# nh2/lz4-frame-conduit

Hardware: AMD Instinct MI355X
Metric: GiB/s end-to-end (compress+decompress), 4 MiB blocks, 1/2/4/8 GPUs vs liblz4 (higher is better)
Workload: dtype u8

## Files before the change

### lz4_frame_conduit_amd/csrc/encode.cuh

```cuda
#pragma once
#include <type_traits>
#include "common.cuh"

namespace lz4f {

constexpr uint32_t MFLIMIT = 12, LASTLIT = 5, MINMATCH = 4;
constexpr uint32_t ENC_POOL_SHORT = 0x200u;

struct ChunkInfo {
    uint32_t nrec;
    uint32_t first_lit;
    uint32_t tail_lit;
    uint32_t body_size;
    uint32_t carry_in;
    uint32_t flags;
    uint64_t out_off;
};

struct EncGeom {
    uint64_t src_size;
    uint64_t first_off;
    uint32_t write_endmark;
    uint32_t block_size;
    uint32_t chunk_size;
    uint32_t chunks_per_block;
    uint32_t n_blocks;
    uint32_t n_chunks;
    uint32_t linked;
    uint32_t block_checksum;
    uint32_t header_size;
    uint8_t  header[20];
    uint32_t max_rec_per_chunk;
    uint64_t rec_pool;
    uint32_t seed_stride;
    uint32_t tiles_per_wg;
    uint32_t e1_solo;
    uint32_t hc_attempts;
    uint32_t hc_lazy;
};

struct EncPlace {
    uint64_t bstart, bend_abs;
    uint64_t cs_abs, ce_abs;
    uint64_t low_abs;
    uint64_t rd_end;
};
__device__ __forceinline__ bool enc_place(const EncGeom& g, uint32_t chunk, EncPlace& pl)
{
    const uint32_t blk = chunk / g.chunks_per_block, cib = chunk % g.chunks_per_block;
    pl.bstart = g.first_off + (uint64_t)blk * g.block_size;
    pl.bend_abs = (pl.bstart + g.block_size < g.src_size) ? pl.bstart + g.block_size : g.src_size;
    pl.cs_abs = pl.bstart + (uint64_t)cib * g.chunk_size;
    if (pl.cs_abs >= pl.bend_abs) return false;
    pl.ce_abs = (pl.cs_abs + g.chunk_size < pl.bend_abs) ? pl.cs_abs + g.chunk_size : pl.bend_abs;
    pl.low_abs = g.linked ? 0 : pl.bstart;
    pl.rd_end = g.src_size;
    return true;
}

__device__ __forceinline__ unsigned long long* rec_ctl(const uint64_t* recs) { return (unsigned long long*)recs; }
__device__ __forceinline__ uint32_t* rec_offs(const uint64_t* recs) { return (uint32_t*)(recs + 8); }
__host__ __device__ __forceinline__ uint64_t rec_pool_at(uint32_t n_chunks) { return 8 + (((uint64_t)n_chunks + 1 + 15) / 16) * 8; }
__device__ __forceinline__ uint64_t* rec_pool_of(const uint64_t* recs, const EncGeom& g) { return (uint64_t*)recs + rec_pool_at(g.n_chunks); }

__device__ __forceinline__ uint32_t len_ext_bytes(uint32_t v) { return v >= 15 ? (v - 15) / 255 + 1 : 0; }
__device__ __forceinline__ uint32_t seq_size(uint32_t lit, uint32_t mlen)
{
    return 1 + len_ext_bytes(lit) + lit + 2 + len_ext_bytes(mlen - MINMATCH);
}
__device__ __forceinline__ uint64_t pack_rec(uint32_t lit, uint32_t mlen, uint32_t off)
{
    return (uint64_t)lit | ((uint64_t)mlen << 24) | ((uint64_t)off << 48);
}

struct uint4_ua { uint32_t x, y, z, w; } __attribute__((packed, aligned(1)));
__device__ __forceinline__ uint32_t ld32(const uint8_t* p) { return *(const u32_ua*)p; }
typedef uint64_t u64_ua __attribute__((aligned(1)));
__device__ __forceinline__ uint64_t ld64_guard(const uint8_t* p, const uint8_t* end)
{
    if (p + 8 <= end) return *(const u64_ua*)p;
    uint64_t v = 0;
    for (int i = 0; i < 8; i++) if (p + i < end) v |= (uint64_t)p[i] << (8 * i);
    return v;
}

constexpr uint32_t E1_TILE = 65536, E1_RING = 2 * E1_TILE, E1_RMASK = E1_RING - 1;
#ifndef E1_SLICE_BYTES
#define E1_SLICE_BYTES 128
#endif
constexpr uint32_t E1_SLICE = E1_SLICE_BYTES, E1_NSLICE = E1_TILE / E1_SLICE, E1_REC_PER_SLICE = E1_SLICE / MINMATCH;
constexpr uint32_t E1_HASH_LOG = 13;
#ifndef E1_WAVES
#define E1_WAVES 16
#endif
#ifdef E1_DEBUG
#define E1DBG(...) __VA_ARGS__
#else
#define E1DBG(...)
#endif
#define E1_DBG_AT (((uint64_t)gridDim.x) * (2 * E1_NSLICE * E1_REC_PER_SLICE))
struct alignas(16) E1Shared {
    uint16_t table[1u << E1_HASH_LOG];
    uint8_t  tags[1u << E1_HASH_LOG];
    uint32_t s_end[2][E1_NSLICE];
    uint8_t  s_n[2][E1_NSLICE];
    uint32_t next, cov;
    uint32_t first;
    uint32_t cur[16];
    uint32_t pieces[2];
    uint32_t mode, hits;
    uint32_t tail_d[2];
    uint32_t idle[64];
    alignas(16) uint8_t ring[E1_RING + 16];
};
static_assert(sizeof(E1Shared) <= 163840, "one workgroup per CU");
static_assert(64 * E1_WAVES >= E1_NSLICE, "a thread per slice when the lists are merged");
#ifndef E1_GRAB
#define E1_GRAB 8
#endif
#ifndef E1_GRAB_D
#define E1_GRAB_D 1
// ... 768 lines not shown
        const uint32_t nr = (c < nch && usable && !(e.word >> 31)) ? ci[c].nrec : 0u;
        uint32_t ts, te;
        const uint32_t ps = wave_excl_scan(nr, ts), pe = wave_excl_scan((nr + IX_STRIDE - 1) / IX_STRIDE, te);
        if (c < g.chunks_per_block) ck[c] = IxChunk{nent + pe, nseq + ps};
        const uint64_t m = __ballot(nr != 0);
        if (m) last = c0 + 63u - (uint32_t)__builtin_clzll(m);
        nseq += ts; nent += te;
    }
    if (lane == 0) {
        if (last != 0xFFFFFFFFu) { ck[last].ent_off |= 0x80000000u; nseq += 1; }
        blocks[b].nseq = nseq; blocks[b].nentries = nent;
    }
}

__global__ __launch_bounds__(1024) void k_build_index(EncGeom g, const ChunkInfo* __restrict__ info, const BlockOut* __restrict__ table,
                                                      const ResultRec* __restrict__ res, void* __restrict__ ix, uint64_t ix_capacity,
                                                      uint32_t blocks_done = 0)
{
    __shared__ uint32_t s_a[1024], s_b[1024];
    __shared__ uint32_t s_carry_a, s_carry_b;
    const uint32_t t = threadIdx.x;
    IxHeader* hd = (IxHeader*)ix;
    IxBlock* blocks = ix_blocks(ix);
    IxChunk* chunks = ix_chunks(ix, g.n_blocks);
    const size_t fixed = ix_entries_at(g.n_blocks, g.chunks_per_block);
    if (ix_capacity < fixed) { if (t == 0 && ix_capacity >= sizeof(IxHeader)) hd->magic = 0; return; }
    const bool usable = res->status == ST_OK;
    for (uint32_t b = t; b < g.n_blocks && !blocks_done; b += 1024) {
        const BlockOut e = table[b];
        const ChunkInfo* ci = info + (uint64_t)b * g.chunks_per_block;
        IxChunk* ck = chunks + (uint64_t)b * g.chunks_per_block;
        const uint32_t nch = (e.dst_size + g.chunk_size - 1) / g.chunk_size;
        uint32_t nseq = 0, nent = 0, last = 0xFFFFFFFFu;
        for (uint32_t c0 = 0; c0 < g.chunks_per_block; c0 += 8) {
            uint32_t nr[8];
#pragma unroll
            for (uint32_t k = 0; k < 8; k++) nr[k] = (c0 + k < nch) ? ci[c0 + k].nrec : 0;
#pragma unroll
            for (uint32_t k = 0; k < 8; k++) {
                const uint32_t c = c0 + k;
                if (c >= g.chunks_per_block) break;
                ck[c] = IxChunk{nent, nseq};
                if (usable && !(e.word >> 31) && nr[k]) { nseq += nr[k]; nent += (nr[k] + IX_STRIDE - 1) / IX_STRIDE; last = c; }
            }
        }
        if (last != 0xFFFFFFFFu) { ck[last].ent_off |= 0x80000000u; nseq += 1; }
        blocks[b].nseq = nseq; blocks[b].nentries = nent;
    }
    __syncthreads();
    if (t == 0) { s_carry_a = 0; s_carry_b = 0; }
    __syncthreads();
    for (uint32_t base = 0; base < g.n_blocks; base += 1024) {
        const uint32_t b = base + t;
        const uint32_t va = (b < g.n_blocks) ? blocks[b].nseq : 0, vb = (b < g.n_blocks) ? blocks[b].nentries : 0;
        s_a[t] = va; s_b[t] = vb;
        __syncthreads();
        for (uint32_t off = 1; off < 1024; off <<= 1) {
            const uint32_t aa = (t >= off) ? s_a[t - off] : 0, ab = (t >= off) ? s_b[t - off] : 0;
            __syncthreads();
            s_a[t] += aa; s_b[t] += ab;
            __syncthreads();
        }
        if (b < g.n_blocks) { blocks[b].seq_base = s_carry_a + s_a[t] - va; blocks[b].entry_base = s_carry_b + s_b[t] - vb; }
        __syncthreads();
        if (t == 1023) { s_carry_a += s_a[1023]; s_carry_b += s_b[1023]; }
        __syncthreads();
    }
    if (t == 0) {
        const bool fits = (uint64_t)s_carry_b * sizeof(IxEntry) <= ix_capacity - fixed;
        *hd = IxHeader{usable && fits ? IX_MAGIC : 0u, g.n_blocks, g.chunks_per_block, s_carry_a, s_carry_b, IX_STRIDE, g.linked ? 1u : 0u, 0u};
    }
}

__device__ __forceinline__ void emit_len_ext(uint8_t* p, uint32_t v )
{
    const uint32_t n255 = v / 255, lane = lane_id();
    for (uint32_t i = lane; i < n255; i += WAVE) p[i] = 255;
    if (lane == 0) p[n255] = (uint8_t)(v - n255 * 255);
}

#ifndef E2_V2
#define E2_V2 1
#endif
template <bool split>
__device__ __forceinline__ void emit_chunk(const uint8_t* __restrict__ src, const EncPlace& pl, const ChunkInfo& ci, const uint64_t* __restrict__ rec,
                                           uint8_t* __restrict__ dst, IxEntry* ent, const uint32_t ent_seq0, const uint32_t ent_last, const uint64_t pay0,
                                           const uint32_t blk, uint4* T0, uint4* T1, const uint32_t sub, const uint32_t nsub)
{
    const uint32_t lane = lane_id();
    const uint64_t bstart = pl.bstart, cs_abs = pl.cs_abs, ce_abs = pl.ce_abs;
    if (ci.flags & 4u) return;
    if (ci.flags & 1u) {
        uint8_t* o = dst + ci.out_off;
        const uint64_t n = ce_abs - cs_abs;
        if (sub) return;
        for (uint64_t off = 0; off < n; off += 1u << 20) {
            const uint32_t m = (uint32_t)((n - off < (1u << 20)) ? n - off : (1u << 20));
            wave_copy_disjoint(o + off, src + cs_abs + off, m);
        }
        return;
    }
    uint64_t lp_off = cs_abs - ci.carry_in;
    uint64_t o_off = ci.out_off;
    auto scan = [&](uint32_t v, uint32_t& total) -> uint32_t {
        uint32_t incl = v;
#pragma unroll
        for (int sft = 1; sft < 64; sft <<= 1) { const uint32_t t = __shfl_up(incl, sft); if ((int)lane >= sft) incl += t; }
        total = __builtin_amdgcn_readlane(incl, 63);
        return incl - v;
    };
    auto find = [&](uint32_t u) -> uint32_t {
        uint32_t j = 0;
#pragma unroll
        for (uint32_t step = 32; step; step >>= 1) { const uint32_t c = j + step; if (T0[c].x <= u) j = c; }
        return j;
    };
    auto put_ext = [&](uint8_t* q, uint32_t v ) {
        const uint32_t n255 = v / 255;
        for (uint32_t i = 0; i < n255; i++) q[i] = 255;
        q[n255] = (uint8_t)(v - n255 * 255);
    };
    if ((uint64_t)ci.nrec * 192 <= ce_abs - cs_abs) {
        uint8_t* o = dst + o_off;
        const uint8_t* lp = src + lp_off;
#if E2_V2
        for (uint32_t r0 = 0; r0 < ci.nrec; r0 += WAVE) {
            const uint32_t rl = r0 + lane;
            const uint64_t xr = rl < ci.nrec ? rec[rl] : 0ull;
            uint32_t vlit = (uint32_t)(xr & 0xFFFFFFu);
            const uint32_t vmlen = (uint32_t)((xr >> 24) & 0xFFFFFFu), voff = (uint32_t)(xr >> 48);
            if (rl == 0) vlit += ci.carry_in;
            const uint32_t vmcode = rl < ci.nrec ? vmlen - MINMATCH : 0u;
            const uint32_t vhb = 1 + len_ext_bytes(vlit), vtb = 2 + len_ext_bytes(vmcode);
            const uint32_t vtoken = ((vlit < 15 ? vlit : 15) << 4) | (vmcode < 15 ? vmcode : 15);
            const uint32_t vlrest = vlit >= 15 ? (vlit - 15) % 255 : 0u, vmrest = vmcode >= 15 ? (vmcode - 15) % 255 : 0u;
            const bool vbig = vhb > WAVE || vtb > WAVE;
            const uint32_t vp1 = (vbig ? 0u : vhb | (vtb << 8)) | (vtoken << 16) | (vlrest << 24), vp2 = voff | (vmrest << 16), vadv = vlit + vmlen;
            const uint32_t nb = ci.nrec - r0 < WAVE ? ci.nrec - r0 : WAVE;
            if constexpr (split) {
                const bool vact = rl < ci.nrec;
                uint32_t tot_sz, tot_adv;
                const uint32_t vso = scan(vact ? vhb + vlit + vtb : 0u, tot_sz), vsa = scan(vact ? vadv : 0u, tot_adv);
                for (uint32_t k = sub; k < nb; k += nsub) {
                    const uint32_t r = r0 + k;
                    const uint32_t lit = (uint32_t)__builtin_amdgcn_readlane((int)vlit, (int)k), so = (uint32_t)__builtin_amdgcn_readlane((int)vso, (int)k);
                    const uint32_t sa = (uint32_t)__builtin_amdgcn_readlane((int)vsa, (int)k);
                    const uint32_t p1 = (uint32_t)__builtin_amdgcn_readlane((int)vp1, (int)k), p2 = (uint32_t)__builtin_amdgcn_readlane((int)vp2, (int)k);
                    const uint32_t hb = p1 & 0xFFu, tb = (p1 >> 8) & 0xFFu, token = (p1 >> 16) & 0xFFu, off = p2 & 0xFFFFu;
                    uint8_t* q = o + so;
                    const uint8_t* ls = lp + sa;
                    if (ent && (r % IX_STRIDE) == 0 && lane == 0) {
                        uint32_t ns = ci.nrec - r < IX_STRIDE ? ci.nrec - r : IX_STRIDE;
                        if (ent_last && r + IX_STRIDE >= ci.nrec) ns += 1;
                        ent[r / IX_STRIDE] = IxEntry{(uint32_t)((uint64_t)(q - dst) - pay0), (uint32_t)((uint64_t)(ls - src) - bstart), ent_seq0 + r, ns | (blk << 8)};
                    }
                    if (hb) {
                        const uint32_t hi = lane < hb - 1 ? lane : hb - 1, ti = lane < tb - 1 ? lane : tb - 1;
                        q[hi] = (uint8_t)(hi == 0 ? token : hi < hb - 1 ? 255u : p1 >> 24);
                        q += hb;
                        wave_copy_disjoint(q, ls, lit);
                        q += lit;
                        q[ti] = (uint8_t)(ti == 0 ? off : ti == 1 ? off >> 8 : ti < tb - 1 ? 255u : p2 >> 16);
                    } else {
                        const uint32_t mcode = (uint32_t)__builtin_amdgcn_readlane((int)vmcode, (int)k);
                        if (lane == 0) *q = (uint8_t)token;
                        q += 1;
                        if (lit >= 15) { emit_len_ext(q, lit - 15); q += len_ext_bytes(lit); }
                        wave_copy_disjoint(q, ls, lit);
                        q += lit;
                        if (lane == 0) { q[0] = (uint8_t)off; q[1] = (uint8_t)(off >> 8); }
                        q += 2;
                        if (mcode >= 15) emit_len_ext(q, mcode - 15);
                    }
                }
                o += tot_sz; lp += tot_adv;
                continue;
            }
            for (uint32_t k = 0; k < nb; k++) {
                const uint32_t r = r0 + k;
                if (ent && (r % IX_STRIDE) == 0 && lane == 0) {
                    uint32_t ns = ci.nrec - r < IX_STRIDE ? ci.nrec - r : IX_STRIDE;
                    if (ent_last && r + IX_STRIDE >= ci.nrec) ns += 1;
                    ent[r / IX_STRIDE] = IxEntry{(uint32_t)((uint64_t)(o - dst) - pay0), (uint32_t)((uint64_t)(lp - src) - bstart), ent_seq0 + r, ns | (blk << 8)};
                }
                const uint32_t lit = (uint32_t)__builtin_amdgcn_readlane((int)vlit, (int)k), adv = (uint32_t)__builtin_amdgcn_readlane((int)vadv, (int)k);
                const uint32_t p1 = (uint32_t)__builtin_amdgcn_readlane((int)vp1, (int)k), p2 = (uint32_t)__builtin_amdgcn_readlane((int)vp2, (int)k);
                const uint32_t hb = p1 & 0xFFu, tb = (p1 >> 8) & 0xFFu, token = (p1 >> 16) & 0xFFu, off = p2 & 0xFFFFu;
                if (hb) {
                    const uint32_t hi = lane < hb - 1 ? lane : hb - 1, ti = lane < tb - 1 ? lane : tb - 1;
                    o[hi] = (uint8_t)(hi == 0 ? token : hi < hb - 1 ? 255u : p1 >> 24);
                    o += hb;
                    wave_copy_disjoint(o, lp, lit);
                    o += lit;
                    o[ti] = (uint8_t)(ti == 0 ? off : ti == 1 ? off >> 8 : ti < tb - 1 ? 255u : p2 >> 16);
                    o += tb;
                } else {
                    const uint32_t mcode = adv - lit - MINMATCH;
                    if (lane == 0) *o = (uint8_t)token;
                    o += 1;
                    if (lit >= 15) { emit_len_ext(o, lit - 15); o += len_ext_bytes(lit); }
                    wave_copy_disjoint(o, lp, lit);
                    o += lit;
                    if (lane == 0) { o[0] = (uint8_t)off; o[1] = (uint8_t)(off >> 8); }
                    o += 2;
                    if (mcode >= 15) { emit_len_ext(o, mcode - 15); o += len_ext_bytes(mcode); }
                }
                lp += adv;
            }
        }
#else
        for (uint32_t r = 0; r < ci.nrec; r++) {
            if (ent && (r % IX_STRIDE) == 0 && lane == 0) {
                uint32_t ns = ci.nrec - r < IX_STRIDE ? ci.nrec - r : IX_STRIDE;
                if (ent_last && r + IX_STRIDE >= ci.nrec) ns += 1;
                ent[r / IX_STRIDE] = IxEntry{(uint32_t)((uint64_t)(o - dst) - pay0), (uint32_t)((uint64_t)(lp - src) - bstart), ent_seq0 + r, ns | (blk << 8)};
            }
            const uint64_t x = rec[r];
            uint32_t lit = (uint32_t)(x & 0xFFFFFFu);
            const uint32_t mlen = (uint32_t)((x >> 24) & 0xFFFFFFu), off = (uint32_t)(x >> 48);
            if (r == 0) lit += ci.carry_in;
            const uint32_t mcode = mlen - MINMATCH;
// ... 73 lines not shown
                const uint8_t* a = on ? sb + (e1.x + o16) : src;
                const b16_ua t = *(const b16_ua*)a;
                pc.a = t.a; pc.b = t.b; pc.c = t.c; pc.d = t.d;
            };
            auto st = [&](const P16& pc, uint32_t dof, bool on) { if (on) *(b16_ua*)(ob + dof) = b16_ua{pc.a, pc.b, pc.c, pc.d}; };
            P16 a0, b0;
            uint32_t da0, db0;
            bool xa0, xb0;
            uint32_t base = 0;
            ld(a0, base + lane, da0, xa0); base += 64;
            for (;;) {
                const bool more_b = base < total;
                ld(b0, base + lane, db0, xb0); base += 64;
                st(a0, da0, xa0);
                if (!more_b) break;
                const bool more_a = base < total;
                ld(a0, base + lane, da0, xa0); base += 64;
                st(b0, db0, xb0);
                if (!more_a) break;
            }
        }
        uint32_t total_b;
        {
            const uint32_t bL = (act && lit < 16) ? lit : 0u;
            const uint32_t P = scan(bL, total_b);
            if (total_b) {
                T0[lane] = uint4{P, bL, 0u, 0u};
                T1[lane] = uint4{sa, so + 1 + le, 0u, 0u};
                __builtin_amdgcn_fence(__ATOMIC_RELEASE, "wavefront"); __builtin_amdgcn_wave_barrier();
            }
        }
        for (uint32_t base = 0; base < total_b; base += 128) {
            uint8_t v[2]; uint32_t dof[2]; bool on[2];
#pragma unroll
            for (int i = 0; i < 2; i++) {
                const uint32_t u = base + 64 * i + lane;
                const uint32_t j = find(u);
                const uint4 e0 = T0[j], e1 = T1[j];
                const uint32_t k = u - e0.x;
                on[i] = u < total_b;
                dof[i] = e1.y + k;
                const uint8_t* a = on[i] ? sb + (e1.x + k) : src;
                v[i] = *a;
            }
#pragma unroll
            for (int i = 0; i < 2; i++) if (on[i]) ob[dof[i]] = v[i];
        }
        __builtin_amdgcn_fence(__ATOMIC_RELEASE, "wavefront"); __builtin_amdgcn_wave_barrier();
        lp_off += tot_adv; o_off += tot_sz;
    }
    if ((ci.flags & 2u) && sub == 0) {
        uint8_t* o = dst + o_off;
        const uint32_t lit = ci.nrec ? ci.tail_lit : ci.tail_lit + ci.carry_in;
        if (lane == 0) *o = (uint8_t)((lit < 15 ? lit : 15) << 4);
        o += 1;
        if (lit >= 15) { emit_len_ext(o, lit - 15); o += len_ext_bytes(lit); }
        wave_copy_disjoint(o, src + lp_off, lit);
    }
}

template <int WAVES_PER_WG, bool split = false>
__global__ __launch_bounds__(64 * WAVES_PER_WG) void k_emit_gather(const uint8_t* __restrict__ src, EncGeom g,
                                                                   const ChunkInfo* __restrict__ info, const uint64_t* __restrict__ recs,
                                                                   uint8_t* __restrict__ dst, const BlockOut* __restrict__ table, void* __restrict__ ix)
{
    __shared__ uint4 s_gt[WAVES_PER_WG][2][64];
    const uint32_t wave = threadIdx.x >> 6;
    const uint32_t chunk = uni(split ? blockIdx.x : blockIdx.x * WAVES_PER_WG + wave);
    const uint32_t sub = split ? wave : 0u, nsub = split ? (uint32_t)WAVES_PER_WG : 1u;
    if (chunk >= g.n_chunks) return;
    EncPlace pl;
    if (!enc_place(g, chunk, pl)) return;
    const uint32_t blk = chunk / g.chunks_per_block;
    const ChunkInfo ci = info[chunk];
    const bool parsed = !(ci.flags & 5u);
    const uint64_t* rec = rec_pool_of(recs, g) + (parsed && ci.nrec ? rec_offs(recs)[chunk] : 0u);
    IxEntry* ent = nullptr; uint32_t ent_seq0 = 0, ent_last = 0; uint64_t pay0 = 0;
    if (parsed && ix && ((const IxHeader*)ix)->magic == IX_MAGIC && ci.nrec) {
        const IxChunk ck = ix_chunks(ix, g.n_blocks)[chunk];
        ent = ix_entries_w(ix, g.n_blocks, g.chunks_per_block) + ix_blocks(ix)[blk].entry_base + (ck.ent_off & 0x7FFFFFFFu);
        ent_seq0 = ck.seq_off; ent_last = ck.ent_off >> 31;
        pay0 = table[blk].src_off;
    }
    emit_chunk<split>(src, pl, ci, rec, dst, ent, ent_seq0, ent_last, pay0, blk, s_gt[wave][0], s_gt[wave][1], sub, nsub);
}

}
```

### lz4_frame_conduit_amd/csrc/encode_batch.cuh

```cuda
#pragma once
#include "common.cuh"
#include "encode.cuh"
#include "encode_solo.cuh"
#include "encode_hc.cuh"
#include "batch_common.cuh"

namespace lz4f {

constexpr uint32_t BC_NONE = BF_NONE;
constexpr uint32_t BC_CHUNK = 65536;
constexpr uint32_t BC_CHUNK_RECS = BC_CHUNK / 4 + 1;

struct BcFrame {
    uint64_t src, len;
    uint64_t dst, win;
    uint64_t rec_at;
    uint64_t fsize;
    uint32_t status, n_blocks, n_chunks;
    uint32_t blk_at, chk_at, pad;
};
struct BcBlk {
    uint64_t src, out;
    uint32_t blen, word, frame, chk_at;
};
// ... 127 lines not shown
    }
}

template <int W>
__global__ __launch_bounds__(64 * W) void k_bc_layout(const BcFrame* __restrict__ frames, uint32_t n_frames, BcBlk* __restrict__ blocks,
                                                      const uint32_t* __restrict__ ctl, ChunkInfo* __restrict__ info)
{
    const uint32_t total = uni(ctl[1]);
    for (uint32_t w = uni(blockIdx.x * W + (threadIdx.x >> 6)); w < total; w += gridDim.x * W) {
        const uint32_t fi = uni(blocks[w].frame);
        if (!bc_blk_live(frames, n_frames, fi, w)) continue;
        const uint32_t blen = uni(blocks[w].blen);
        const uint32_t word = layout_block_chunks(info + uni(blocks[w].chk_at), (blen + BC_CHUNK - 1) / BC_CHUNK, blen);
        if (lane_id() == 0) blocks[w].word = word;
    }
}

template <int W>
__global__ __launch_bounds__(64 * W) void k_bc_frames(uint8_t* dst, BcFrame* __restrict__ frames, uint32_t n_frames, BcPrefs pf, BcBlk* __restrict__ blocks,
                                                      ChunkInfo* __restrict__ info, ResultRec* __restrict__ results)
{
    const uint32_t i = uni(blockIdx.x * W + (threadIdx.x >> 6));
    if (i >= n_frames) return;
    const uint32_t lane = lane_id();
    const uint32_t status = uni(frames[i].status), nb = uni(frames[i].n_blocks), nc = uni(frames[i].n_chunks);
    const uint32_t blk_at = uni(frames[i].blk_at), chk_at = uni(frames[i].chk_at);
    const uint64_t len = uni64(frames[i].len), d0 = uni64(frames[i].dst), win = uni64(frames[i].win);
    auto flg_with = [&](bool csize) { return make_flg(!pf.linked, pf.block_checksum, csize, pf.content_checksum, pf.dict_id != 0); };
    if (status != 0) {
        if (lane == 0) results[i] = ResultRec{0ull, 0ull, status, 0u, 0xFFFFFFFFu, flg_with(pf.content_size) | (LZ4F_MI355X_PATH_BATCH << 12)};
        return;
    }
    const uint32_t flg = flg_with(pf.content_size && len != 0), flags = flg | (LZ4F_MI355X_PATH_BATCH << 12);
    const uint32_t hs = frame_head_size(flg);
    uint64_t at = d0 + hs;
    for (uint32_t b0 = 0; b0 < nb; b0 += WAVE) {
        const uint32_t b = b0 + lane;
        const uint32_t bytes = b < nb ? 4u + (blocks[blk_at + b].word & 0x7FFFFFFFu) + 4u * pf.block_checksum : 0u;
        uint32_t sum;
        const uint32_t before = wave_excl_scan(bytes, sum);
        if (b < nb) blocks[blk_at + b].out = at + before + 4;
        at += sum;
    }
    const uint64_t fsize = at - d0 + 4 + (pf.content_checksum ? 4 : 0);
    const bool fits = fsize <= win;
    __threadfence();
    if (fits) {
        if (lane == 0) {
            uint8_t h[20];
            const uint32_t n = frame_head_write(h, flg, pf.bsid, len, pf.dict_id);
            for (uint32_t q = 0; q < n; q++) dst[d0 + q] = h[q];
        }
        for (uint32_t b = lane; b < nb; b += WAVE) st32le(dst + blocks[blk_at + b].out - 4, blocks[blk_at + b].word);
        if (lane < 4) dst[at + lane] = 0;
    }
    const uint32_t cpb = pf.block_size / BC_CHUNK;
    for (uint32_t c = lane; c < nc; c += WAVE) {
        ChunkInfo* ci = info + chk_at + c;
        if (!fits) { ci->flags |= 4u; continue; }
        const uint32_t b = c / cpb, cib = c % cpb;
        const BcBlk e = blocks[blk_at + b];
        ci->out_off = (e.word >> 31) ? e.out + (uint64_t)cib * BC_CHUNK : e.out + ci->out_off;
    }
    if (lane == 0) {
        frames[i].fsize = fsize;
        if (!fits) frames[i].status = ST_DSTSMALL;
        results[i] = ResultRec{fits ? fsize : 0ull, len, fits ? (uint32_t)ST_OK : (uint32_t)ST_DSTSMALL, nb, 0xFFFFFFFFu, flags};
    }
}

template <int W>
__global__ __launch_bounds__(64 * W) void k_bc_emit(const uint8_t* __restrict__ src, uint8_t* __restrict__ dst, const BcFrame* __restrict__ frames,
                                                    uint32_t n_frames, const BcChunk* __restrict__ chunks, const uint32_t* __restrict__ ctl,
                                                    const ChunkInfo* __restrict__ info, const uint64_t* __restrict__ pool)
{
    __shared__ uint4 s_gt[W][2][64];
    const uint32_t wv = uni(threadIdx.x >> 6);
    const uint32_t total = uni(ctl[0]);
    for (uint32_t w = uni(blockIdx.x * W + wv); w < total; w += gridDim.x * W) {
        const BcChunk e = chunks[w];
        if (!bc_chunk_live(frames, n_frames, uni(e.frame), w)) continue;
        const EncPlace pl = bc_place_of(e);
        const ChunkInfo ci = info[w];
        emit_chunk<false>(src, pl, ci, pool + uni64(e.rec_at), dst, nullptr, 0u, 0u, 0ull, 0u, s_gt[wv][0], s_gt[wv][1], 0u, 1u);
        __builtin_amdgcn_fence(__ATOMIC_RELEASE, "wavefront"); __builtin_amdgcn_wave_barrier();
    }
}

template <int W, bool LANE4>
__global__ __launch_bounds__(64 * W) void k_bc_blockck(uint8_t* dst, const BcFrame* __restrict__ frames, uint32_t n_frames, const BcBlk* __restrict__ blocks,
                                                       const uint32_t* __restrict__ ctl)
{
    __shared__ __attribute__((aligned(16))) uint32_t park[W][LANE4 ? XXH_PARK / 4 : 1];
    const uint32_t wv = uni(threadIdx.x >> 6);
    const uint32_t total = uni(ctl[1]);
    for (uint32_t w = uni(blockIdx.x * W + wv); w < total; w += gridDim.x * W) {
        const uint32_t fi = uni(blocks[w].frame);
        if (!bc_blk_live(frames, n_frames, fi, w)) continue;
        const uint64_t off = uni64(blocks[w].out);
        const uint32_t n = uni(blocks[w].word) & 0x7FFFFFFFu;
        uint32_t h;
        if constexpr (LANE4) h = lane4_xxh32(dst + off, n, park[wv]); else h = wave_xxh32(dst + off, n);
        if (lane_id() == 0) st32le(dst + off + n, h);
    }
}

template <int W>
__global__ __launch_bounds__(64 * W) void k_bc_content(const uint8_t* __restrict__ src, uint8_t* dst, const BcFrame* __restrict__ frames, uint32_t n_frames)
{
    __shared__ __attribute__((aligned(16))) uint32_t park[W][XXH_PARK / 4];
    const uint32_t wv = uni(threadIdx.x >> 6);
    const uint32_t i = uni(blockIdx.x * W + wv);
    if (i >= n_frames) return;
    if (uni(frames[i].status) != 0) return;
    const uint32_t h = lane4_xxh32(src + uni64(frames[i].src), uni64(frames[i].len), park[wv]);
    if (lane_id() == 0) st32le(dst + uni64(frames[i].dst) + uni64(frames[i].fsize) - 4, h);
}

}
```

### lz4_frame_conduit_amd/csrc/engine.hip

```cpp
#include <hip/hip_runtime.h>
#include <stdarg.h>
#include <stdio.h>
#include <stdlib.h>
#include <string.h>

#include <algorithm>
#include <mutex>
#include <vector>

#include "engine.hpp"
#include "frame_dev.cuh"
#include "decode_batch.cuh"
#include "encode_batch.cuh"
#include "measure_batch.cuh"

using namespace lz4f;

static_assert(sizeof(ChunkInfo) == 32, "chunk info layout");
static_assert(sizeof(BatchFrame) == 80 && sizeof(BatchBlk) == 40, "batch workspace layout");
static_assert(sizeof(BatchCore) == 64 && sizeof(MeasBlk) == 24, "batch measure workspace layout");
static_assert(sizeof(BcFrame) == 72 && sizeof(BcBlk) == 32 && sizeof(BcChunk) == 64, "batch encode workspace layout");

namespace lz4f {

static thread_local char t_err[512] = "";
static thread_local int t_device = -1;

void set_last_error(const char* fmt, ...)
{
    va_list ap; va_start(ap, fmt); vsnprintf(t_err, sizeof(t_err), fmt, ap); va_end(ap);
}
const char* last_error() { return t_err; }

static int grow(void** p, size_t* cap, size_t n, bool pinned)
{
    if (n <= *cap) return 0;
    const size_t want = n + n / 8 + 4096;
    if (*p) (void)(pinned ? hipHostFree(*p) : hipFree(*p));
    *p = nullptr; *cap = 0;
    const hipError_t e = pinned ? hipHostMalloc(p, want, hipHostMallocDefault) : hipMalloc(p, want);
    if (e != hipSuccess) { set_last_error("%s(%zu) failed: %s", pinned ? "hipHostMalloc" : "hipMalloc", want, hipGetErrorString(e)); *p = nullptr; return 1; }
    *cap = want;
    return 0;
}
int DevBuf::ensure(size_t n) { return grow(&p, &cap, n, false); }
int PinBuf::ensure(size_t n) { return grow(&p, &cap, n, true); }
void DevBuf::release() { if (p) (void)hipFree(p); p = nullptr; cap = 0; }
void PinBuf::release() { if (p) (void)hipHostFree(p); p = nullptr; cap = 0; }

int selected_device()
{
    if (t_device < 0) {
        const char* s = getenv("LZ4F_MI355X_DEVICE");
        t_device = s ? atoi(s) : 0;
    }
    return t_device;
}

uint32_t pick_chunk_size(uint32_t block_size)
{
    const uint32_t c = 64u << 10;
    return block_size < c ? block_size : c;
}

}
void lz4f_mi355x_engine::Switches::read()
{
    auto on = [](const char* n) { return getenv(n) != nullptr; };
    auto num = [](const char* n, int lo, int hi, int dflt) { const char* v = getenv(n); if (!v) return dflt; const int k = atoi(v); return k >= lo && k <= hi ? k : dflt; };
    no_index = on("LZ4F_MI355X_NO_INDEX");
    no_selfindex = on("LZ4F_MI355X_NO_SELFINDEX");
    no_resolve = on("LZ4F_MI355X_NO_RESOLVE");
    no_trace = on("LZ4F_MI355X_NO_TRACE");
    no_doubling = on("LZ4F_MI355X_NO_DOUBLING");
    trace_always = on("LZ4F_MI355X_TRACE_ALWAYS");
    no_groups = on("LZ4F_MI355X_NO_GROUPS");
    no_window = on("LZ4F_MI355X_NO_WINDOW");
    serial_walk = on("LZ4F_MI355X_SERIAL_WALK");
    no_trailer = on("LZ4F_MI355X_NO_TRAILER");
    no_density_probe = on("LZ4F_MI355X_NO_DENSITY_PROBE");
    no_spx = on("LZ4F_MI355X_NO_SPX");
    no_overlap = on("LZ4F_MI355X_NO_OVERLAP");
    no_content_check = on("LZ4F_MI355X_NO_CONTENT_CHECK");
    prof = on("LZ4F_MI355X_PROF");
    e1_sync = on("LZ4F_MI355X_E1_SYNC");
    no_selffeed = on("LZ4F_MI355X_NO_SELFFEED");
    dense_mode = (unsigned)num("LZ4F_MI355X_DENSE_MODE", 0, 2, 0);
    group_kib = (unsigned)num("LZ4F_MI355X_GROUP_KIB", 64, 4096, 0);
    if (group_kib & (group_kib - 1)) group_kib = 0;
    feed_round = (unsigned)num("LZ4F_MI355X_FEED_ROUND", 17, 4096, 0);
    chain_gate = num("LZ4F_MI355X_CHAIN_GATE", 1, (1 << 20) - 1, 0);
    decode_mode = 0; if (const char* v = getenv("LZ4F_MI355X_DECODE")) decode_mode = v[0];
    e1_run = (unsigned)num("LZ4F_MI355X_E1_RUN", 1, 4096, 0);
    e1_solo = 0; if (const char* v = getenv("LZ4F_MI355X_E1_SOLO")) e1_solo = (unsigned)atoi(v);
    if (on("LZ4F_MI355X_DETERMINISTIC")) e1_solo |= 1u;
    wait_ticks = 0; if (const char* v = getenv("LZ4F_MI355X_WAIT_TICKS")) { unsigned long long a = 0; if (sscanf(v, "%llu", &a) == 1) wait_ticks = a; }
    dblk_lds = (unsigned)num("LZ4F_MI355X_DBLK_LDS", 1, 150, 0) << 10;
    recs_per_tile = (unsigned)num("LZ4F_MI355X_RECS_PER_TILE", 1, 16385, 0);
    hc_attempts = (unsigned)num("LZ4F_MI355X_HC_ATTEMPTS", 1, 65536, 0);
    hc_lazy = (unsigned)num("LZ4F_MI355X_HC_LAZY", 1, 2, 0);
    seed = 2; if (const char* v = getenv("LZ4F_MI355X_SEED")) { unsigned a = 0; if (sscanf(v, "%u", &a) == 1 && a >= 1 && a <= 64) seed = a; }
}
namespace lz4f {
size_t new_engine(lz4f_mi355x_engine** out, int device, void* stream, bool borrow)
{
    int n = 0;
    hipError_t e = hipGetDeviceCount(&n);
    if (e != hipSuccess || n <= 0) {
        set_last_error("no usable HIP device (hipGetDeviceCount: %s, count %d): liblz4f_mi355x has no CPU fallback", hipGetErrorString(e), n);
        return make_err(LZ4F_ERROR_GENERIC);
    }
    if (device < 0 || device >= n) { set_last_error("device %d out of range (%d devices)", device, n); return make_err(LZ4F_ERROR_GENERIC); }
    HIP_TRY(hipSetDevice(device));
    lz4f_mi355x_engine* en = new lz4f_mi355x_engine();
    en->device = device;
    en->sw.read();
    if (borrow) { en->stream = stream; en->own_stream = false; }
    else {
        hipStream_t s;
        hipError_t e2 = hipStreamCreateWithFlags(&s, hipStreamNonBlocking);
        if (e2 != hipSuccess) { delete en; set_last_error("hipStreamCreate failed: %s", hipGetErrorString(e2)); return make_err(LZ4F_ERROR_GENERIC); }
        en->stream = s; en->own_stream = true;
    }
    *out = en;
    return 0;
}

namespace {
struct EnginePool {
    std::mutex mu;
    std::vector<lz4f_mi355x_engine*> idle;
    ~EnginePool() { drain(); }
    void drain()
    {
        std::vector<lz4f_mi355x_engine*> v;
        { std::lock_guard<std::mutex> g(mu); v.swap(idle); }
        for (auto* e : v) delete e;
    }
};
EnginePool& pool() { static EnginePool p; return p; }
}

size_t acquire_engine(lz4f_mi355x_engine** out, int device)
{
    if (device < 0) device = selected_device();
    {
        EnginePool& p = pool();
        std::lock_guard<std::mutex> g(p.mu);
        for (size_t i = 0; i < p.idle.size(); i++)
            if (p.idle[i]->device == device) { *out = p.idle[i]; p.idle.erase(p.idle.begin() + i); return 0; }
    }
    return new_engine(out, device, nullptr, false);
}
void release_engine(lz4f_mi355x_engine* e)
{
    if (!e) return;
    EnginePool& p = pool();
    std::lock_guard<std::mutex> g(p.mu);
    p.idle.push_back(e);
}
void release_idle_engines() { pool().drain(); }

}

lz4f_mi355x_engine::~lz4f_mi355x_engine()
{
    (void)hipSetDevice(device);
    (void)hipStreamSynchronize((hipStream_t)stream);
    desc.release(); seqcnt.release(); spx.release(); selfix.release(); selfcnt.release(); postab.release(); pdbuf.release(); tight.release();
// ... 27 lines not shown

size_t lz4f_mi355x_engine::sync()
{
    HIP_TRY(hipSetDevice(device));
    HIP_TRY(hipStreamSynchronize((hipStream_t)stream));
    if (aux_pending && aux_stream) { HIP_TRY(hipStreamSynchronize((hipStream_t)aux_stream)); aux_pending = false; }
    return 0;
}

static unsigned long long* g_prof = nullptr;
static unsigned long long* prof_buf()
{
    if (!g_prof) { if (hipMalloc(&g_prof, 1024) != hipSuccess) return nullptr; (void)hipMemset(g_prof, 0, 1024); (void)hipMemset(g_prof + 70, 0xFF, 8); (void)hipMemset(g_prof + 75, 0xFF, 8); }
    return g_prof;
}
extern "C" __attribute__((visibility("default"))) int lz4f_mi355x_debug_prof(unsigned long long* out128)
{
    if (!prof_buf()) return 1;
    (void)hipDeviceSynchronize();
    const int rc = hipMemcpy(out128, g_prof, 1024, hipMemcpyDeviceToHost) == hipSuccess ? 0 : 2;
#ifdef DB_PROF
    { unsigned long long z[32] = {0}; (void)hipMemcpyFromSymbol(out128 + 96, HIP_SYMBOL(lz4f::g_dbprof), sizeof(z)); (void)hipMemcpyToSymbol(HIP_SYMBOL(lz4f::g_dbprof), z, sizeof(z)); }
#endif
    (void)hipMemset(g_prof, 0, 1024); (void)hipMemset(g_prof + 70, 0xFF, 8); (void)hipMemset(g_prof + 75, 0xFF, 8);
    return rc;
}

static uint32_t device_cus(int device)
{
    static int cus[64];
    const unsigned d = (unsigned)device % 64;
    if (!cus[d]) { int v = 0; if (hipDeviceGetAttribute(&v, hipDeviceAttributeMultiprocessorCount, device) != hipSuccess || v < 1) v = 256; cus[d] = v; }
    return (uint32_t)cus[d];
}


struct EncShape { uint32_t chunk, chunks_per_block; uint64_t n_blocks; };
static EncShape enc_shape(uint64_t payload, uint32_t block_size)
{
    const uint32_t chunk = pick_chunk_size(block_size);
    return EncShape{chunk, block_size / chunk, (payload + block_size - 1) / block_size};
}
static size_t index_capacity(uint64_t payload, const EncShape& s)
{
    return ix_entries_at((uint32_t)s.n_blocks, s.chunks_per_block) + ix_typical_entries(payload, (uint32_t)(s.n_blocks * s.chunks_per_block)) * sizeof(IxEntry);
}

static uint64_t rec_pool_records(uint32_t n_chunks, uint32_t max_rec_per_chunk, unsigned per_tile)
{
    const uint64_t worst = (uint64_t)(n_chunks + 1) * max_rec_per_chunk;
    uint64_t want = (uint64_t)(n_chunks + 1) * (per_tile ? per_tile : 12288u);
    if (want < 64ull * max_rec_per_chunk) want = 64ull * max_rec_per_chunk;
    if (want > worst) want = worst;
    if (want > 0xFFFFFFF0ull) want = 0xFFFFFFF0ull;
    return want;
}

struct lz4f_mi355x_engine::EncodePlan {
    bool too_large;
    EncGeom g;
    enum Finder { E1_SHARED, E1_SOLO, HASH_CHAIN } finder;
    uint32_t e1_wgs;
    bool layout_small, e2_split;
    bool xxh_lane4;
    bool inband;
    size_t index_cap;
    size_t info_bytes, recs_bytes, blk_bytes, table_bytes, res_bytes, e1_scratch_bytes, ixtmp_bytes;
};

lz4f_mi355x_engine::EncodePlan lz4f_mi355x_engine::encode_plan(const CompressJob& j, const Switches& sw, uint32_t cus, bool inband, size_t index_cap)
{
    EncodePlan p; memset(&p, 0, sizeof(p));
    EncGeom& g = p.g;
    const uint64_t payload = j.src_size - j.first_off;
    const EncShape s = enc_shape(payload, j.block_size);
    if (s.n_blocks > 0x7FFFFFFFull / s.chunks_per_block) { p.too_large = true; return p; }
    g.src_size = j.src_size; g.first_off = j.first_off; g.write_endmark = j.endmark ? (j.content_checksum ? 2 : 1) : 0;
    g.block_size = j.block_size; g.chunk_size = s.chunk; g.chunks_per_block = s.chunks_per_block;
    g.n_blocks = (uint32_t)s.n_blocks; g.n_chunks = g.n_blocks * g.chunks_per_block;
    g.linked = j.linked; g.block_checksum = j.block_checksum;
    g.header_size = j.header_size; memcpy(g.header, j.header, j.header_size);
    g.max_rec_per_chunk = g.chunk_size / 4 + 1;
    g.seed_stride = sw.seed;
    const bool hc = j.level >= 3;
    p.finder = hc ? EncodePlan::HASH_CHAIN : ((sw.e1_solo & 1u) && !(sw.e1_solo & 4u)) ? EncodePlan::E1_SOLO : EncodePlan::E1_SHARED;
    if (hc) {
        const HcLevel hl = hc_level(j.level);
        g.hc_attempts = sw.hc_attempts ? sw.hc_attempts : hl.attempts;
        g.hc_lazy = sw.hc_lazy ? sw.hc_lazy : hl.lazy;
    }
    g.rec_pool = rec_pool_records(g.n_chunks, g.max_rec_per_chunk, ((sw.e1_solo & 1u) || hc) ? 16385u : sw.recs_per_tile);
    if (g.n_chunks) {
        uint32_t run = g.n_chunks / cus; run = run < 1 ? 1 : run > 64 ? 64 : run;
        if ((g.n_chunks + run - 1) / run > 1024) run = (g.n_chunks + 1023) / 1024;
        if (sw.e1_run) run = sw.e1_run;
        g.tiles_per_wg = run;
        g.e1_solo = sw.e1_solo;
        p.e1_wgs = (g.n_chunks + run - 1) / run;
        p.e1_scratch_bytes = (size_t)p.e1_wgs * 2 * E1_NSLICE * E1_REC_PER_SLICE * 8 + 2048;
    }
    p.layout_small = g.n_blocks <= LAYOUT_SMALL_BLOCKS && g.n_chunks <= LAYOUT_SMALL_CHUNKS; p.e2_split = g.n_chunks <= 512;
    p.xxh_lane4 = g.n_blocks < XXH_LANE4_BELOW;
    p.inband = inband;
    p.index_cap = inband ? index_capacity(payload, s) + 64 : index_cap;
    p.ixtmp_bytes = inband ? p.index_cap + 64 : 0;
    p.info_bytes = (size_t)(g.n_chunks + 1) * sizeof(ChunkInfo); p.recs_bytes = (size_t)(rec_pool_at(g.n_chunks) + g.rec_pool) * 8;
    p.blk_bytes = (size_t)(g.n_blocks + 1) * 4; p.table_bytes = (size_t)(g.n_blocks + 1) * sizeof(BlockOut);
    p.res_bytes = sizeof(ResultRec) + sizeof(TrailerPlan) + 64;
    return p;
}

#ifdef E1_DEBUG
static void e1_debug_dump(hipStream_t st, const uint8_t* counters)
{
    unsigned long long d[256]; if (hipStreamSynchronize(st) == hipSuccess && hipMemcpy(d, counters, 2048, hipMemcpyDeviceToHost) == hipSuccess) {
                for (int w = 0; w < 16; w += 5) { unsigned long long* x = d + 16 + w * 8; if (x[6]) fprintf(stderr, "E1 wave %d: per tile cycles: merge %llu parse %llu waitB1 %llu dma-issue %llu dma-wait %llu waitB2 %llu (%llu tiles)\n", w, x[0]/x[6], x[1]/x[6], x[2]/x[6], x[3]/x[6], x[4]/x[6], x[5]/x[6], x[6]); unsigned long long* f = d + 160 + w * 6; fprintf(stderr, "   parse: dequeue %llu cycles x %llu, probe step %llu cycles x %llu, hit %llu cycles x %llu (per tile)\n", f[3] ? f[0]/f[3] : 0, f[3]/x[6], f[4] ? f[1]/f[4] : 0, f[4]/x[6], f[5] ? f[2]/f[5] : 0, f[5]/x[6]); }
                fprintf(stderr, "E1 dense passes (workgroup 0): %llu, matches taken %llu, positions advanced %llu; one-match steps because: hit in B %llu, mode not dense %llu, step != 1 %llu, first match long %llu\n", d[13], d[14], d[15], d[4], d[5], d[6], d[7]);
                fprintf(stderr, "E1 debug: bounds hit: dequeue %llu, probe %llu, backward %llu, forward %llu; probe ip/last %llx step/slice %llx; back room/nb %llx; fwd mp/fw %llx end_lim/d %llx\n", d[0], d[1], d[2], d[3], d[8], d[9], d[10], d[11], d[12]); }
}
#endif

size_t lz4f_mi355x_engine::enc_workspaces(const EncodePlan& p, bool own_table)
{
    if (ixtmp.ensure(p.ixtmp_bytes) || res.ensure(p.res_bytes) || info.ensure(p.info_bytes) || recs.ensure(p.recs_bytes) || blk_bytes.ensure(p.blk_bytes) ||
        (own_table && table.ensure(p.table_bytes)) || e1_scratch.ensure(p.e1_scratch_bytes))
        return make_err(LZ4F_ERROR_allocation_failed);
    return 0;
}

size_t lz4f_mi355x_engine::enc_find(const CompressJob& j, const EncodePlan& p)
{
    hipStream_t st = (hipStream_t)stream; const EncGeom& g = p.g;
#ifdef E1_DEBUG
    uint8_t* const counters = (uint8_t*)e1_scratch.p + p.e1_scratch_bytes - 2048;
    (void)hipMemsetAsync(counters, 0, 2048, st);
#endif
    if (recs_ctl_clean != recs.p) { HIP_TRY(hipMemsetAsync(recs.p, 0, 64, st)); }
    recs_ctl_clean = nullptr;
    if (p.finder == EncodePlan::HASH_CHAIN)
        hipLaunchKernelGGL(k_find_matches_hc, dim3(g.n_chunks), dim3(64 * HC_WAVES), 0, st, j.d_src, g, (ChunkInfo*)info.p, (uint64_t*)recs.p);
    else if (p.finder == EncodePlan::E1_SOLO)
        hipLaunchKernelGGL((k_find_matches_solo<1>), dim3(g.n_chunks), dim3(64), 0, st, j.d_src, g, (ChunkInfo*)info.p, (uint64_t*)recs.p);
    else
        hipLaunchKernelGGL(k_find_matches, dim3(p.e1_wgs), dim3(64 * E1_WAVES), 0, st, j.d_src, g, (ChunkInfo*)info.p, (uint64_t*)recs.p, (uint64_t*)e1_scratch.p);
    if (sw.e1_sync) (void)hipStreamSynchronize(st);
#ifdef E1_DEBUG
    e1_debug_dump(st, counters);
#endif
    return 0;
}

void lz4f_mi355x_engine::enc_layout(const EncodePlan& p, uint8_t* d_dst, uint64_t dst_cap, ResultRec* rec, BlockOut* tbl, void* d_index)
{
    constexpr int W = 4;
    hipStream_t st = (hipStream_t)stream; const EncGeom& g = p.g;
    if (p.layout_small)
        hipLaunchKernelGGL(k_layout_small, dim3(1), dim3(1024), 0, st, g, (ChunkInfo*)info.p, tbl, (uint32_t*)blk_bytes.p, d_dst, dst_cap, rec, (const uint64_t*)recs.p);
    else {
        if (g.n_blocks) hipLaunchKernelGGL((k_layout_blocks<W>), dim3((g.n_blocks + W - 1) / W), dim3(64 * W), 0, st, g, (ChunkInfo*)info.p, tbl, (uint32_t*)blk_bytes.p);
        hipLaunchKernelGGL(k_layout_scan, dim3(1), dim3(1024), 0, st, g, tbl, (const uint32_t*)blk_bytes.p, d_dst, dst_cap, rec, (const uint64_t*)recs.p);
        if (g.n_chunks) hipLaunchKernelGGL(k_layout_chunks, dim3((g.n_chunks + 255) / 256), dim3(256), 0, st, g, (ChunkInfo*)info.p, (const BlockOut*)tbl, d_dst, (const ResultRec*)rec);
    }
    if (g.n_chunks) recs_ctl_clean = recs.p;
    if (d_index) {
        if (g.n_blocks) hipLaunchKernelGGL((k_index_blocks<W>), dim3((g.n_blocks + W - 1) / W), dim3(64 * W), 0, st, g, (const ChunkInfo*)info.p, (const BlockOut*)tbl, (const ResultRec*)rec, d_index, (uint64_t)p.index_cap);
        hipLaunchKernelGGL(k_build_index, dim3(1), dim3(1024), 0, st, g, (const ChunkInfo*)info.p, (const BlockOut*)tbl, (const ResultRec*)rec, d_index, (uint64_t)p.index_cap, 1u);
// ... 826 lines not shown
```

### lz4_frame_conduit_amd/csrc/engine.hpp

```cpp
#pragma once
#include <stddef.h>
#include <stdint.h>
#include <functional>
#include <string>
#include <vector>

#include "../../include/lz4f_mi355x.h"
#include "records.hpp"

namespace lz4f {

inline size_t make_err(int code) { return (size_t)-(ptrdiff_t)code; }
inline bool   is_err(size_t v) { return v > make_err(LZ4F_ERROR_maxCode); }
const char*   err_name(size_t v);
void          set_last_error(const char* fmt, ...);
const char*   last_error();

struct Xxh32State {
    uint32_t total_len, large, v[4], memsize;
    uint8_t  mem[16];
    void reset(uint32_t seed = 0);
    void update(const void* data, size_t len);
    uint32_t digest() const;
};
uint32_t xxh32_host(const void* data, size_t len, uint32_t seed = 0);

size_t block_size_of(unsigned blockSizeID);
size_t write_frame_header(uint8_t* dst, const LZ4F_preferences_t& p);
size_t compress_bound_internal(size_t srcSize, const LZ4F_preferences_t* prefs, size_t alreadyBuffered);
struct ParsedHeader { LZ4F_frameInfo_t info; size_t header_size; size_t max_block; };
size_t parse_frame_header(const uint8_t* src, size_t n, ParsedHeader* out);

struct DevBuf {
    void* p = nullptr; size_t cap = 0;
    int ensure(size_t n);
    void release();
};
struct PinBuf {
    void* p = nullptr; size_t cap = 0;
    int ensure(size_t n);
    void release();
};

#define HIP_TRY(expr)                                                                                   \
    do {                                                                                                \
        hipError_t e_ = (expr);                                                                         \
        if (e_ != hipSuccess) {                                                                         \
            lz4f::set_last_error("%s failed: %s (%s:%d)", #expr, hipGetErrorString(e_), __FILE__, __LINE__);  \
            return lz4f::make_err(LZ4F_ERROR_GENERIC);                                                  \
        }                                                                                               \
    } while (0)

}

struct lz4f_mi355x_engine {
    int   device = 0;
    void* stream = nullptr;
    bool  own_stream = false;
    lz4f::DevBuf info, recs, table, blk_bytes, res, bad;
    lz4f::DevBuf ixtmp;
    lz4f::DevBuf walkbuf;
    lz4f::DevBuf density;
    lz4f::DevBuf e1_scratch;
    lz4f::DevBuf spx;
    lz4f::DevBuf selfix, selfcnt;
    lz4f::DevBuf pdbuf;
    lz4f::DevBuf tight;
    lz4f::DevBuf postab;
    lz4f::DevBuf desc, seqcnt;
    lz4f::DevBuf d_in, d_out;
    lz4f::DevBuf bframes, btable;
    lz4f::DevBuf mframes, mtable;
    lz4f::DevBuf cframes, cblocks, cchunks;
    lz4f::PinBuf h_in, h_out, h_small;
    struct Switches {
        bool no_index, no_selfindex, no_resolve, no_trace, no_doubling, trace_always, no_groups, no_window, serial_walk, no_trailer, no_content_check, no_density_probe, no_spx, no_overlap, prof, e1_sync, no_selffeed;
        unsigned dense_mode;
        unsigned group_kib;
        unsigned feed_round;
        int chain_gate; char decode_mode; unsigned e1_run, e1_solo, seed, dblk_lds, recs_per_tile, hc_attempts, hc_lazy; unsigned long long wait_ticks;
        void read();
    } sw;
    void*  recs_ctl_clean = nullptr;
    size_t ix_seq_cap = 0;
    bool  timing = false;
    void* ev[24] = {nullptr};
    bool  ev_used[12] = {false};
    void  tick(int slot, bool end, void* on_stream = nullptr);
    void* aux_stream = nullptr; void* ev_fork = nullptr; void* ev_join = nullptr;
    bool  aux_ready();
    bool  aux_pending = false;

    struct CompressJob {
        const uint8_t* d_src; uint64_t src_size; uint64_t first_off;
        uint32_t block_size; bool linked; bool block_checksum; bool endmark;
        bool content_checksum;
        uint8_t header[20]; uint32_t header_size;
        int level;
    };
    static CompressJob make_compress_job(const uint8_t* d_src, uint64_t src_size, uint64_t first_off, uint32_t block_size, bool linked, bool block_checksum,
                                         int level, const LZ4F_preferences_t* frame = nullptr);
    size_t launch_compress(const CompressJob& j, uint8_t* d_dst, uint64_t dst_cap, lz4f_mi355x_result* d_res, lz4f_mi355x_block* d_table,
                           void* d_index = nullptr, size_t index_cap = 0);
    struct DecompressJob {
        const uint8_t* d_frame; uint64_t frame_cap; uint8_t* d_dst; uint64_t dst_cap; uint64_t hist0;
        void* d_index; size_t index_size;
        uint32_t block_size; bool linked; bool block_checksum;
        bool content_checksum;
        const lz4f_mi355x_block* d_table; uint32_t n_blocks;
        bool table_in_place;
        lz4f_mi355x_block* table_direct;
        uint32_t max_blocks;
        const uint64_t* hint_list; uint32_t hint_n;
        uint32_t ix_seqs, ix_entries;
    };
    size_t launch_decompress(const DecompressJob& j, lz4f_mi355x_result* d_res);
    size_t sync();

    size_t compress_blocks_host(const uint8_t* src, size_t n, const uint8_t* hist, size_t hist_len,
                                uint32_t block_size, bool linked, bool block_checksum, uint8_t* dst, size_t dst_cap, size_t* written, int level = 0);
    size_t slab_compress(const uint8_t* src, size_t n, const uint8_t* hist, size_t hist_len, uint32_t block_size, bool linked, bool block_checksum,
                         bool src_pinned, size_t* size, int level = 0);
    size_t slab_fetch(uint8_t* dst, size_t size, size_t d_off, bool dst_pinned);
    size_t compress_block_pinned(const uint8_t* pin_src, size_t hist_len, size_t n, uint32_t block_size, bool linked, bool block_checksum,
                                 uint8_t* pin_dst, size_t dst_cap, size_t* size, int level = 0);
    size_t slab_decode(const uint8_t* frame_part, size_t part_len, const std::vector<lz4f_mi355x_block>& entries, const lz4f::ParsedHeader& ph,
                       const uint8_t* hist, size_t hist_len, bool src_pinned, size_t* got, uint8_t* fetch_to = nullptr, size_t fetch_room = 0);
    size_t decompress_block_host(const uint8_t* payload, uint32_t csize, bool bck, const uint8_t* hist, size_t hist_len,
                                 uint8_t* dst, uint32_t dst_cap, bool linked, uint32_t block_size, uint32_t* decoded);

    ~lz4f_mi355x_engine();

private:
    struct EncodePlan;
    static EncodePlan encode_plan(const CompressJob& j, const Switches& sw, uint32_t cus, bool inband, size_t index_cap);
    size_t enc_workspaces(const EncodePlan& p, bool own_table);
    size_t enc_find(const CompressJob& j, const EncodePlan& p);
    void   enc_layout(const EncodePlan& p, uint8_t* d_dst, uint64_t dst_cap, lz4f::ResultRec* rec, lz4f::BlockOut* tbl, void* d_index);
    void   enc_emit(const CompressJob& j, const EncodePlan& p, uint8_t* d_dst, const lz4f::ResultRec* rec, lz4f::BlockOut* tbl, void* d_index);
    void   enc_tail(const CompressJob& j, const EncodePlan& p, uint8_t* d_dst, uint64_t dst_cap, lz4f::ResultRec* rec, const lz4f::BlockOut* tbl, const void* d_index);

    struct DecodePlan {
        bool given, begin_small;
        uint32_t n_max, n_ix;
        enum Walk { WALK_NONE, WALK_TRAILER, WALK_PARALLEL, WALK_SEEDED, WALK_SERIAL } walk;
        char mode;
        bool ix_by_trailer;
        bool self_index;
        bool windowed, small, relay;
        uint32_t group;
        uint64_t wait_ticks;
    };
    struct IndexSrc {
        enum From { GIVEN, TRAILER, HEADER, SELF_LINKED, SPX } from = GIVEN;
        void* d = nullptr; size_t size = 0;
        uint32_t seqs = 0, entries = 0;
    };
    struct IxRoute { bool selffed, doubling; uint32_t gate; };
    static DecodePlan decode_plan(const DecompressJob& j, const Switches& sw, uint32_t cus);
// ... 40 lines not shown
```

Before: 748.8.

## Emit sequences wave-parallel with 16-byte literal copy units in non-split encoder

Adds a new default path in the non-split emit kernel. Instead of walking records one by one, each wave prefix-scans output sizes, input advances and 16-byte literal units across 64 records. All lanes then copy literal runs in 16-byte loads and stores distributed across records, and token, offset and length bytes are written per lane in parallel. This targets the serial per-record walk and the underutilised lanes on short literals. The cost is extra scans, ballots and bpermutes, plus overlapping or clamped stores. The old walk stays available via an environment switch, and the batch encoder still uses it.

```diff
diff --git a/lz4_frame_conduit_amd/csrc/encode.cuh b/lz4_frame_conduit_amd/csrc/encode.cuh
--- a/lz4_frame_conduit_amd/csrc/encode.cuh
+++ b/lz4_frame_conduit_amd/csrc/encode.cuh
@@ -37,6 +37,7 @@
     uint32_t e1_solo;
     uint32_t hc_attempts;
     uint32_t hc_lazy;
+    uint32_t emit_walk;
 };
 
 struct EncPlace {
@@ -971,10 +972,11 @@
 #ifndef E2_V2
 #define E2_V2 1
 #endif
+constexpr uint32_t E2_STEP_RUNS = 8;
 template <bool split>
 __device__ __forceinline__ void emit_chunk(const uint8_t* __restrict__ src, const EncPlace& pl, const ChunkInfo& ci, const uint64_t* __restrict__ rec,
                                            uint8_t* __restrict__ dst, IxEntry* ent, const uint32_t ent_seq0, const uint32_t ent_last, const uint64_t pay0,
-                                           const uint32_t blk, uint4* T0, uint4* T1, const uint32_t sub, const uint32_t nsub)
+                                           const uint32_t blk, uint4* T0, uint4* T1, const uint32_t sub, const uint32_t nsub, const bool walk)
 {
     const uint32_t lane = lane_id();
     const uint64_t bstart = pl.bstart, cs_abs = pl.cs_abs, ce_abs = pl.ce_abs;
@@ -1026,6 +1028,88 @@
             const bool vbig = vhb > WAVE || vtb > WAVE;
             const uint32_t vp1 = (vbig ? 0u : vhb | (vtb << 8)) | (vtoken << 16) | (vlrest << 24), vp2 = voff | (vmrest << 16), vadv = vlit + vmlen;
             const uint32_t nb = ci.nrec - r0 < WAVE ? ci.nrec - r0 : WAVE;
+            if constexpr (!split) if (!walk) {
+                const bool vact = rl < ci.nrec;
+                const bool vunit = vact && !vbig && vlit >= 16, vbyte = vact && !vbig && vlit != 0 && vlit < 16;
+                const uint32_t vu = vunit ? (vlit + 15) >> 4 : 0u, vsz = vact ? vhb + vlit + vtb : 0u, vad = vact ? vadv : 0u;
+                const uint32_t iP = dpp_incl_scan_add(vu), iso = dpp_incl_scan_add(vsz), isa = dpp_incl_scan_add(vad);
+                const uint32_t U = (uint32_t)__builtin_amdgcn_readlane((int)iP, 63), tot_sz = (uint32_t)__builtin_amdgcn_readlane((int)iso, 63);
+                const uint32_t tot_adv = (uint32_t)__builtin_amdgcn_readlane((int)isa, 63);
+                const uint32_t vP = iP - vu, vso = iso - vsz, vsa = isa - vad;
+                if (U) {
+                    const uint32_t vsb = vsa - vP * 16u, vdb = vso + vhb - vP * 16u, vlim = vlit + vP * 16u;
+                    uint64_t rem = __ballot(vunit);
+                    uint32_t ub = 0, jlast = 0;
+                    struct P16 { uint32_t a, b, c, d; };
+                    auto ld = [&](P16& pc, uint32_t& dof) {
+                        uint32_t ue = ub + WAVE < U ? ub + WAVE : U;
+                        uint32_t u = ub + lane;
+                        uint32_t jl = jlast;
+                        for (uint32_t cnt = 0; rem; cnt++) {
+                            const uint32_t j = (uint32_t)__builtin_ctzll(rem);
+                            const uint32_t Pj = (uint32_t)__builtin_amdgcn_readlane((int)vP, (int)j);
+                            if (Pj >= ue) break;
+                            if (cnt == E2_STEP_RUNS) { ue = Pj; break; }
+                            jl = u >= Pj ? j : jl;
+                            jlast = j;
+                            if (Pj + (uint32_t)__builtin_amdgcn_readlane((int)vu, (int)j) > ue) break;
+                            rem &= rem - 1;
+                        }
+                        u = u < ue ? u : ue - 1;
+                        const uint32_t sb = (uint32_t)__builtin_amdgcn_ds_bpermute((int)(jl << 2), (int)vsb);
+                        const uint32_t db = (uint32_t)__builtin_amdgcn_ds_bpermute((int)(jl << 2), (int)vdb);
+                        const uint32_t lim = (uint32_t)__builtin_amdgcn_ds_bpermute((int)(jl << 2), (int)vlim);
+                        uint32_t a16 = u * 16u;
+                        a16 = (a16 + 16u > lim) ? lim - 16u : a16;
+                        dof = db + a16;
+                        const b16_ua t = *(const b16_ua*)(lp + (uint32_t)(sb + a16));
+                        pc.a = t.a; pc.b = t.b; pc.c = t.c; pc.d = t.d;
+                        ub = ue;
+                    };
+                    auto st = [&](const P16& pc, uint32_t dof) { *(b16_ua*)(o + dof) = b16_ua{pc.a, pc.b, pc.c, pc.d}; };
+                    P16 a0, b0;
+                    uint32_t da0, db0;
+                    do {
+                        ld(a0, da0);
+                        ld(b0, db0);
+                        __builtin_amdgcn_sched_barrier(0);
+                        st(a0, da0);
+                        st(b0, db0);
+                    } while (ub < U);
+                }
+                if (vact && !vbig) {
+                    uint8_t* q = o + vso;
+                    q[0] = (uint8_t)vtoken;
+                    if (vlit >= 15) { for (uint32_t i = 1; i + 1 < vhb; i++) q[i] = 255; q[vhb - 1] = (uint8_t)vlrest; }
+                    q += vhb + vlit;
+                    q[0] = (uint8_t)voff; q[1] = (uint8_t)(voff >> 8);
+                    if (vmcode >= 15) { for (uint32_t i = 2; i + 1 < vtb; i++) q[i] = 255; q[vtb - 1] = (uint8_t)vmrest; }
+                }
+                if (ent && vact && (rl % IX_STRIDE) == 0) {
+                    uint32_t ns = ci.nrec - rl < IX_STRIDE ? ci.nrec - rl : IX_STRIDE;
+                    if (ent_last && rl + IX_STRIDE >= ci.nrec) ns += 1;
+                    ent[rl / IX_STRIDE] = IxEntry{(uint32_t)((uint64_t)(o - dst) + vso - pay0), (uint32_t)((uint64_t)(lp - src) + vsa - bstart), ent_seq0 + rl, ns | (blk << 8)};
+                }
+                for (uint32_t i = 0; i < 15 && __ballot(vbyte && i < vlit); i++)
+                    if (vbyte && i < vlit) o[vso + vhb + i] = lp[vsa + i];
+                for (uint64_t mb = __ballot(vact && vbig); mb; mb &= mb - 1) {
+                    const int k = __builtin_ctzll(mb);
+                    const uint32_t lit = (uint32_t)__builtin_amdgcn_readlane((int)vlit, k), mcode = (uint32_t)__builtin_amdgcn_readlane((int)vmcode, k);
+                    const uint32_t token = (uint32_t)__builtin_amdgcn_readlane((int)vtoken, k), off = (uint32_t)__builtin_amdgcn_readlane((int)voff, k);
+                    uint8_t* q = o + (uint32_t)__builtin_amdgcn_readlane((int)vso, k);
+                    const uint8_t* ls = lp + (uint32_t)__builtin_amdgcn_readlane((int)vsa, k);
+                    if (lane == 0) *q = (uint8_t)token;
+                    q += 1;
+                    if (lit >= 15) { emit_len_ext(q, lit - 15); q += len_ext_bytes(lit); }
+                    wave_copy_disjoint(q, ls, lit);
+                    q += lit;
+                    if (lane == 0) { q[0] = (uint8_t)off; q[1] = (uint8_t)(off >> 8); }
+                    q += 2;
+                    if (mcode >= 15) emit_len_ext(q, mcode - 15);
+                }
+                o += tot_sz; lp += tot_adv;
+                continue;
+            }
             if constexpr (split) {
                 const bool vact = rl < ci.nrec;
                 uint32_t tot_sz, tot_adv;
@@ -1265,7 +1349,7 @@
         ent_seq0 = ck.seq_off; ent_last = ck.ent_off >> 31;
         pay0 = table[blk].src_off;
     }
-    emit_chunk<split>(src, pl, ci, rec, dst, ent, ent_seq0, ent_last, pay0, blk, s_gt[wave][0], s_gt[wave][1], sub, nsub);
-}
-
-}
+    emit_chunk<split>(src, pl, ci, rec, dst, ent, ent_seq0, ent_last, pay0, blk, s_gt[wave][0], s_gt[wave][1], sub, nsub, g.emit_walk != 0);
+}
+
+}
diff --git a/lz4_frame_conduit_amd/csrc/encode_batch.cuh b/lz4_frame_conduit_amd/csrc/encode_batch.cuh
--- a/lz4_frame_conduit_amd/csrc/encode_batch.cuh
+++ b/lz4_frame_conduit_amd/csrc/encode_batch.cuh
@@ -233,7 +233,7 @@
         if (!bc_chunk_live(frames, n_frames, uni(e.frame), w)) continue;
         const EncPlace pl = bc_place_of(e);
         const ChunkInfo ci = info[w];
-        emit_chunk<false>(src, pl, ci, pool + uni64(e.rec_at), dst, nullptr, 0u, 0u, 0ull, 0u, s_gt[wv][0], s_gt[wv][1], 0u, 1u);
+        emit_chunk<false>(src, pl, ci, pool + uni64(e.rec_at), dst, nullptr, 0u, 0u, 0ull, 0u, s_gt[wv][0], s_gt[wv][1], 0u, 1u, true);
         __builtin_amdgcn_fence(__ATOMIC_RELEASE, "wavefront"); __builtin_amdgcn_wave_barrier();
     }
 }
diff --git a/lz4_frame_conduit_amd/csrc/engine.hip b/lz4_frame_conduit_amd/csrc/engine.hip
--- a/lz4_frame_conduit_amd/csrc/engine.hip
+++ b/lz4_frame_conduit_amd/csrc/engine.hip
@@ -85,6 +85,7 @@
     prof = on("LZ4F_MI355X_PROF");
     e1_sync = on("LZ4F_MI355X_E1_SYNC");
     no_selffeed = on("LZ4F_MI355X_NO_SELFFEED");
+    emit_walk = on("LZ4F_MI355X_EMIT_WALK");
     dense_mode = (unsigned)num("LZ4F_MI355X_DENSE_MODE", 0, 2, 0);
     group_kib = (unsigned)num("LZ4F_MI355X_GROUP_KIB", 64, 4096, 0);
     if (group_kib & (group_kib - 1)) group_kib = 0;
@@ -278,6 +279,7 @@
     g.header_size = j.header_size; memcpy(g.header, j.header, j.header_size);
     g.max_rec_per_chunk = g.chunk_size / 4 + 1;
     g.seed_stride = sw.seed;
+    g.emit_walk = sw.emit_walk ? 1u : 0u;
     const bool hc = j.level >= 3;
     p.finder = hc ? EncodePlan::HASH_CHAIN : ((sw.e1_solo & 1u) && !(sw.e1_solo & 4u)) ? EncodePlan::E1_SOLO : EncodePlan::E1_SHARED;
     if (hc) {
diff --git a/lz4_frame_conduit_amd/csrc/engine.hpp b/lz4_frame_conduit_amd/csrc/engine.hpp
--- a/lz4_frame_conduit_amd/csrc/engine.hpp
+++ b/lz4_frame_conduit_amd/csrc/engine.hpp
@@ -74,7 +74,7 @@
     lz4f::DevBuf cframes, cblocks, cchunks;
     lz4f::PinBuf h_in, h_out, h_small;
     struct Switches {
-        bool no_index, no_selfindex, no_resolve, no_trace, no_doubling, trace_always, no_groups, no_window, serial_walk, no_trailer, no_content_check, no_density_probe, no_spx, no_overlap, prof, e1_sync, no_selffeed;
+        bool no_index, no_selfindex, no_resolve, no_trace, no_doubling, trace_always, no_groups, no_window, serial_walk, no_trailer, no_content_check, no_density_probe, no_spx, no_overlap, prof, e1_sync, no_selffeed, emit_walk;
         unsigned dense_mode;
         unsigned group_kib;
         unsigned feed_round;
```

Result: slower. 707.6 (-5.5%).
